# reallinshengxiang/Implementation-of-Rank-Algorithm-for-Mainstream-Recommender-Systems

Hardware: AMD Instinct MI355X
Metric: forward samples/sec at batch 4096 (DCN, DIN, BST) on 1/2/4/8 MI355X (higher is better)
Workload: dtype f32; 1 GPU; configs[2]: DIN forward, seq_len 50, emb_dim 32, batch 4096 per GPU; model=DIN, global_batch=4096, seq_len=50, emb_dim=32, tables=wechat_algo_data1 sizes (feedid 106445 rows), mode=eval, inputs resident in HBM, interaction_weights=frozen, parallelism=replicas x1, step=prepared single-kernel launch (rk_din_plan_launch)

## Files before the change

implementation-of-rank-algorithm-for-mainstream-recommender-systems_amd/csrc/din_fused.hip:

```cpp
#include <cstdlib>
#include <new>

#include "mlp_core.h"
#include "mlp_stream.h"

namespace rk {

typedef __attribute__((address_space(3))) void lds_void;
typedef __attribute__((address_space(1))) void glb_void;

#ifndef RK_DIN_HOIST
#define RK_DIN_HOIST 0
#endif

constexpr int kDinSegs = 32;
constexpr int kDinSegLdsOff = 528;
struct DinSegs {
  rk_segment s[kDinSegs];
};

struct DinArgs {
  DinSegs segs;
  uint8_t col_seg[256], col_off[256];
  const float* att_image;
  int nseg, width, q_col, att_col, l2_col0;
  const float* key_table;
  int64_t key_rows, ld_key;
  const int64_t* seq;
  int64_t ld_seq;
  int T;
  const int64_t* seq_len;
  int64_t batch;
  const float *w1, *b1, *w2, *b2, *w3, *b3;
  int use_softmax;
  int bal_nb;
  float* l2_part;
  unsigned* l2_count;
  float* l2_out;
  float l2_scale;
  uint32_t* flags;
  rk_mlp_layer L[RK_MLP_MAX_LAYERS];
  int nl;
  rk_epilogue head;
  int ld0, ld1;
  int epi_off;
  const float* epi_image;
};

template <int H>
struct DinLds {
  static constexpr int LDH = H + 4;
  static constexpr int WK = 0, WQK = WK + 64 * LDH, WQ = WQK + 64 * LDH, W2 = WQ + 64 * LDH;
  static constexpr int B1 = W2 + 32 * 68, B2 = B1 + 64, W3 = B2 + 32, U = W3 + 32, NORM = U + 16 * 64;
  static constexpr int BUF0 = NORM + 16;
};

#ifdef RK_DIN_PHASES
constexpr int kDinPhaseWG = 1024;
constexpr int kDinMarks = 9;
__device__ unsigned long long g_din_ts[kDinPhaseWG][kDinMarks];
__device__ unsigned long long g_din_wave[kDinPhaseWG][16];
__shared__ unsigned long long s_din_ts[kDinMarks];
__shared__ unsigned long long s_din_wave[16];
#define DIN_TS(i)                                \
  do {                                           \
    if (tid == 0) s_din_ts[i] = wall_clock64();  \
  } while (0)
#define DIN_TS_ENTRY()                                              \
  do {                                                              \
    if (tid < kDinMarks) s_din_ts[tid] = tid ? 0 : wall_clock64();  \
  } while (0)
__device__ __forceinline__ void din_marks_flush(int tid) {
  __syncthreads();
  if (blockIdx.x < kDinPhaseWG) {
    if (tid < kDinMarks) g_din_ts[blockIdx.x][tid] = s_din_ts[tid];
    if (tid < 16) g_din_wave[blockIdx.x][tid] = s_din_wave[tid];
  }
}
#else
#define DIN_TS(i) \
  do {            \
  } while (0)
#define DIN_TS_ENTRY() DIN_TS(0)
#endif

constexpr int kDinBalMax = 8;
constexpr int kDinBalClasses = 17;

__device__ __forceinline__ int wave_incl_scan(int v) {
  v += __builtin_amdgcn_update_dpp(0, v, 0x111, 0xf, 0xf, true);
  v += __builtin_amdgcn_update_dpp(0, v, 0x112, 0xf, 0xf, true);
  v += __builtin_amdgcn_update_dpp(0, v, 0x114, 0xf, 0xf, true);
  v += __builtin_amdgcn_update_dpp(0, v, 0x118, 0xf, 0xf, true);
  v += __builtin_amdgcn_update_dpp(0, v, 0x142, 0xa, 0xf, false);
  v += __builtin_amdgcn_update_dpp(0, v, 0x143, 0xc, 0xf, false);
  return v;
}

template <int H>
constexpr int din_pre_chunks() {
  return (16 + 34 + H) / 16 < 7 ? (16 + 34 + H) / 16 : 7;
}
static __shared__ unsigned s_din_rows_ready;
__device__ __forceinline__ void din_l2_handoff(float* l2_part, unsigned* l2_count, float* l2_out, float l2_scale,
                                               int64_t batch, const float* norms, int lane) {
  unsigned prev = 0;
  if (lane == 0) {
    float t = 0.f;
    for (int w = 0; w < kMlpRows; ++w) t += norms[w];
    const float old = __hip_atomic_exchange(l2_part + blockIdx.x, t, __ATOMIC_RELAXED, __HIP_MEMORY_SCOPE_AGENT);
    unsigned one = 1u;
    asm volatile("s_waitcnt vmcnt(0)" : "+v"(one) : "v"(old) : "memory");
    prev = __hip_atomic_fetch_add(l2_count, one, __ATOMIC_RELAXED, __HIP_MEMORY_SCOPE_AGENT);
  }
  prev = __builtin_amdgcn_readfirstlane(prev);
  if (prev == gridDim.x - 1) {
    float t = 0.f;
    for (int i = lane; i < (int)gridDim.x; i += 64)
      t += __hip_atomic_fetch_add(l2_part + i, 0.0f, __ATOMIC_RELAXED, __HIP_MEMORY_SCOPE_AGENT);
    t = wave_sum(t);
    if (lane == 0) {
      l2_out[0] = l2_scale * (t / (float)batch);
      __hip_atomic_store(l2_count, 0u, __ATOMIC_RELAXED, __HIP_MEMORY_SCOPE_AGENT);
    }
  }
#ifdef RK_DIN_PHASES
  if (lane == 0) s_din_ts[8] = wall_clock64();
#endif
}

struct DinL2Args {
  float* part;
  unsigned* count;
  float* out;
  float scale;
  int64_t batch;
};
static __shared__ DinL2Args s_din_l2;

template <class P, int H, bool WAIT, bool DMA>
struct DinRowsReady {
  static constexpr int kSideLayer = P::NL - 1;
  static_assert(P::NL >= 2 && P::nt(P::NL - 1) < kMlpWaves && P::tpw(P::NL - 1, kMlpWaves - 1) == 0,
                "the side layer leaves the last wave without a tile");
  __device__ void issue() const {}
  __device__ void operator()() const {
    if constexpr (DMA) asm volatile("s_waitcnt vmcnt(%0)" ::"n"(RK_STREAM_RING) : "memory");
    if constexpr (WAIT) {
      while (__builtin_amdgcn_readfirstlane(__hip_atomic_load(&s_din_rows_ready, __ATOMIC_RELAXED,
                                                              __HIP_MEMORY_SCOPE_WORKGROUP)) < (unsigned)kMlpWaves)
        __builtin_amdgcn_s_sleep(1);
      asm volatile("" ::: "memory");
    }
  }
  __device__ void side() const {
    if (__builtin_amdgcn_readfirstlane((int)threadIdx.x >> 6) != kMlpWaves - 1) return;
    const DinL2Args l2 = s_din_l2;
    if (!l2.part) return;
    extern __shared__ __attribute__((aligned(16))) float sm[];
    din_l2_handoff(l2.part, l2.count, l2.out, l2.scale, l2.batch, sm + DinLds<H>::NORM, (int)threadIdx.x & 63);
  }
};

template <int H, int NIT, class P, int KS = 0>
__global__ __launch_bounds__(kMlpThreads) void din_forward_kernel(DinArgs a) {
  using Ly = DinLds<H>;
  constexpr int NQ = H / 8;
  extern __shared__ __attribute__((aligned(16))) float sm[];
  float* const buf0 = sm + Ly::BUF0;
  float* const buf1 = buf0 + kMlpRows * a.ld0;
  uint8_t* const col_seg = reinterpret_cast<uint8_t*>(buf1 + kMlpRows * a.ld1);
  uint8_t* const col_off = col_seg + 256;
  rk_segment* const lsegs = reinterpret_cast<rk_segment*>(col_seg + kDinSegLdsOff);

  const int tid = threadIdx.x, lane = tid & 63, wave = tid >> 6;
  const int l32 = lane & 31, half = lane >> 5, hk = 4 * half;
  DIN_TS_ENTRY();

  static_assert(sizeof(rk_segment) % 4 == 0, "segment descriptor of whole words");
  const int seg_words = a.nseg * (int)(sizeof(rk_segment) / 4);
  uint8_t cs_v = 255, co_v = 0;
  int sw_v = 0;
  if (tid < 256) {
    cs_v = a.col_seg[tid];
    co_v = a.col_off[tid];
  }
  if (tid < seg_words) sw_v = reinterpret_cast<const int*>(&a.segs)[tid];

  const int64_t m0 = (int64_t)blockIdx.x * kMlpRows;
  const int ntiles_all = (a.T + 15) / 16;
  auto clamp_len = [&](int64_t len) { return len <= 0 ? 0 : (len >= a.T ? a.T : (int)len); };
  auto tiles_of = [&](int lc) { return lc ? (lc + 15) >> 4 : (a.use_softmax ? ntiles_all : 0); };
  int64_t* const kpre0 = reinterpret_cast<int64_t*>(col_seg + kDinSegLdsOff + sizeof(rk_segment) * kDinSegs);
  int64_t* const s_rows = kpre0 + 64 * kMlpRows;
  unsigned long long* const s_mask = reinterpret_cast<unsigned long long*>(s_rows + kMlpRows);
  int rows;
  int my_tiles = -1;
  int64_t my_len = 0;
  int64_t lv[NIT > 0 ? NIT : 1];
  int u0 = 0, UB = (int)a.batch, UG = (int)gridDim.x, ugl = (int)blockIdx.x;
  if constexpr (NIT == 1) {
    const int j = (int)blockIdx.x / (kMlpThreads / kMlpRows);
    u0 = j * kMlpThreads;
    UB = min(kMlpThreads, (int)(a.batch - u0));
    UG = (UB + kMlpRows - 1) / kMlpRows;
    ugl = (int)blockIdx.x - j * (kMlpThreads / kMlpRows);
  }
  if constexpr (NIT > 0) {
#pragma unroll
    for (int r = 0; r < NIT; ++r) {
      const int64_t i = u0 + tid + kMlpThreads * r;
      lv[r] = a.seq_len[i < a.batch ? i : a.batch - 1];
    }
  } else {
    rows = (int)min<int64_t>(kMlpRows, a.batch - m0);
    if (lane < rows) {
      my_len = a.seq_len[m0 + lane];
      my_tiles = tiles_of(clamp_len(my_len));
    }
  }

  static_assert(Ly::U % 4 == 0, "image of whole float4s");
  constexpr int kImg4 = Ly::U / 4, kPer = (kImg4 + kMlpThreads - 1) / kMlpThreads;
  f32x4_t v[kPer];
  if (a.att_image) {
#pragma unroll
    for (int r = 0; r < kPer; ++r) {
      const int i = tid + r * kMlpThreads;
      if (i < kImg4) v[r] = reinterpret_cast<const f32x4_t*>(a.att_image)[i];
    }
  }
  using Epi = std::conditional_t<std::is_void_v<P>, NoStage, StreamEpi<std::conditional_t<std::is_void_v<P>, StreamPlanK128, P>>>;
  Epi epi_img;
  const bool epi_dma = a.epi_image != nullptr;
#ifndef RK_DIN_EXP_NOEPI
  if constexpr (!std::is_void_v<P>)
    if (!epi_dma) epi_img.load(a.L, tid);
#endif
  auto image_to_lds = [&]() {
#ifndef RK_DIN_EXP_NOEPI
    if constexpr (!std::is_void_v<P>)
      if (!epi_dma) epi_img.store(sm + a.epi_off, tid);
#endif
    if (a.att_image) {
#pragma unroll
      for (int r = 0; r < kPer; ++r) {
        const int i = tid + r * kMlpThreads;
        if (i < kImg4) reinterpret_cast<f32x4_t*>(sm)[i] = v[r];
      }
    } else {
      for (int i = tid; i < 64 * H; i += kMlpThreads) {
        const int j = i / H, h = i % H;
        const float* r = a.w1 + (int64_t)j * 4 * H;
        sm[Ly::WQ + j * Ly::LDH + h] = r[h] + r[2 * H + h];
        sm[Ly::WK + j * Ly::LDH + h] = r[H + h] - r[2 * H + h];
        sm[Ly::WQK + j * Ly::LDH + h] = r[3 * H + h];
      }
      for (int i = tid; i < 32 * 64; i += kMlpThreads) sm[Ly::W2 + (i / 64) * 68 + (i % 64)] = a.w2[i];
      if (tid < 64) sm[Ly::B1 + tid] = a.b1[tid];
      if (tid < 32) {
        sm[Ly::B2 + tid] = a.b2[tid];
        sm[Ly::W3 + tid] = a.w3[tid];
      }
    }
  };
  if (tid < 256) {
    col_seg[tid] = cs_v;
    col_off[tid] = co_v;
  }
  if (tid < seg_words) reinterpret_cast<int*>(lsegs)[tid] = sw_v;
  uint32_t* flags = a.flags;

  const int wp = pad64(a.width);
  constexpr int kColIt = 4;
  int64_t kidx = 0;
  float cval[kColIt];
  auto gather_issue = [&](int64_t bs, bool lv_, int nt_) {
    if (lv_ && lane < 16 * nt_ && lane < a.T) kidx = a.seq[bs * a.ld_seq + lane];
    int64_t cidx[kColIt];
    int cseg[kColIt];
#pragma unroll
    for (int i = 0; i < kColIt; ++i) {
      const int c = lane + 64 * i;
      cseg[i] = (lv_ && c < a.width) ? col_seg[c] : 255;
      cidx[i] = bs;
      if (cseg[i] != 255 && lsegs[cseg[i]].idx) cidx[i] = lsegs[cseg[i]].idx[bs * lsegs[cseg[i]].idx_stride];
    }
#pragma unroll
    for (int i = 0; i < kColIt; ++i) {
      const int c = lane + 64 * i;
      cval[i] = 0.f;
      if (cseg[i] != 255) {
        const rk_segment& g = lsegs[cseg[i]];
        if (g.idx && (cidx[i] < 0 || cidx[i] >= g.rows))
          flag_oob(flags);
        else
          cval[i] = g.src[cidx[i] * g.src_ld + col_off[c]];
      }
    }
  };
  auto gather_store = [&](float* rowp, int64_t* kslot) {
    kslot[lane] = kidx;
#pragma unroll
    for (int i = 0; i < kColIt; ++i) {
      const int c = lane + 64 * i;
      if (c < wp) rowp[c] = cval[i];
    }
  };

  if constexpr (NIT == 0) {
    asm volatile("s_waitcnt lgkmcnt(0)\n\ts_barrier" ::: "memory");
    const int tiles_w = __builtin_amdgcn_readlane(my_tiles, wave);
    gather_issue(m0 + wave, wave < rows, tiles_w);
    image_to_lds();
// ... 633 lines not shown
```

implementation-of-rank-algorithm-for-mainstream-recommender-systems_amd/csrc/mlp_core.h:

```cpp
#pragma once

#include <type_traits>

#include "common.h"

namespace rk {

#ifndef RK_MLP_EPI_PRIO
#define RK_MLP_EPI_PRIO 1
#endif
#ifndef RK_MLP_SYNC
#define RK_MLP_SYNC 1
#endif
#ifndef RK_MLP_EARLY_RING
#define RK_MLP_EARLY_RING 0
#endif
#ifndef RK_MLP_EP_LANES16
#define RK_MLP_EP_LANES16 0
#endif
#ifndef RK_MLP_UNIFORM_PREP
#define RK_MLP_UNIFORM_PREP 0
#endif

constexpr int kMlpRows = 16;
// ... 191 lines not shown
        const int cA = min(c + 1, kchunks - 1);
#pragma unroll
        for (int t = 0; t < RT; ++t)
          ab[(s + 1) & 1][t] = *reinterpret_cast<const f32x4_t*>(arow + 16 * t * ldin + 16 * cA);
        __builtin_amdgcn_sched_barrier(0);
#pragma unroll
        for (int e = 0; e < 4; ++e)
#pragma unroll
          for (int j = 0; j < TPW; ++j)
#pragma unroll
            for (int t = 0; t < RT; ++t) acc[j][t] = mfma16(ab[s & 1][t][e], P.ring[s * TPW + j][e], acc[j][t]);
        if constexpr (decltype(refill)::value) {
          const int cn = min(c + PD, kchunks - 1);
#pragma unroll
          for (int j = 0; j < TPW; ++j)
            P.ring[s * TPW + j] = *reinterpret_cast<const f32x4_t*>(P.wrow[j] + kFragStep * cn);
        }
      }
      __builtin_amdgcn_sched_barrier(0);
    }
  };
  int c0 = 0;
  for (; c0 + PD < kchunks; c0 += PD) {
    cycle(c0, PD, std::true_type{});
#if RK_MLP_SYNC
    if ((c0 + PD) % kMlpSyncChunks == 0) mlp_sync_barrier();
#endif
  }
  if (kchunks - c0 == PD) {
    cycle(c0, PD, std::false_type{});
  } else {
    cycle(c0, kchunks - c0, std::false_type{});
    __builtin_amdgcn_s_waitcnt(0x0F70);
  }
  next();

#ifdef RK_MLP_PHASES
  if (wave == 0 && lane == 0) s_mlp_marks[dbg_mark] = clock64() - dbg_t0;
  if (lane == 0 && dbg_mark / 4 < 4) s_mlp_wave_marks[dbg_mark / 4][wave][0] = (unsigned)(clock64() - dbg_t0);
#endif
#if RK_MLP_EPI_PRIO
  __builtin_amdgcn_s_setprio(2);
#endif
  float* const store = STORE ? L.store : nullptr;
  const int64_t ld_store = L.ld_store;
  auto epilogue = [&](auto DICE, auto RES) {
#pragma unroll
    for (int j = 0; j < TPW; ++j) {
      const int n = 16 * (wave + kMlpWaves * j) + li;
      const bool real = n < L.n;
      const ColEpi ep = ep_bcast(P.ep[j], lane);
      float res[RT][4];
#pragma unroll
      for (int t = 0; t < RT; ++t)
#pragma unroll
        for (int r = 0; r < 4; ++r) res[t][r] = RES ? out[(16 * t + (lane >> 4) * 4 + r) * ldout + n] : 0.f;
#pragma unroll
      for (int t = 0; t < RT; ++t)
#pragma unroll
        for (int r = 0; r < 4; ++r) {
          const int row = 16 * t + (lane >> 4) * 4 + r;
          const float v = col_apply(L, ep, DICE, acc[j][t][r], RES, res[t][r]);
          const float z = real ? v : 0.f;
          out[row * ldout + n] = z;
          if constexpr (STORE)
            if (store && real && row < rows) store[(m0 + row) * ld_store + n] = z;
        }
    }
  };
  const bool dice = L.act == RK_ACT_DICE;
  if (L.residual != 0) {
    if (dice)
      epilogue(std::true_type{}, std::true_type{});
    else
      epilogue(std::false_type{}, std::true_type{});
  } else {
    if (dice)
      epilogue(std::true_type{}, std::false_type{});
    else
      epilogue(std::false_type{}, std::false_type{});
  }
#ifdef RK_MLP_PHASES
  if (lane == 0 && dbg_mark / 4 < 4) s_mlp_wave_marks[dbg_mark / 4][wave][1] = (unsigned)(clock64() - dbg_t0);
#endif
}

__device__ __forceinline__ void mlp_lds_barrier() { asm volatile("s_waitcnt lgkmcnt(0)\n\ts_barrier" ::: "memory"); }

struct NoStage {
  __device__ void issue() const {}
  __device__ void operator()() const {}
  __device__ void side() const {}
};
template <class I, class F>
struct TwoPhaseStage {
  I i;
  F f;
  __device__ void issue() { i(); }
  __device__ void operator()() { f(); }
  __device__ void side() {}
};
template <class E, class I, class F, class S>
struct StagedStage {
  static constexpr bool kEarly = true;
  E e;
  I i;
  F f;
  S s;
  __device__ void early() { e(); }
  __device__ void issue() { i(); }
  __device__ void operator()() { f(); }
  __device__ void side() { s(); }
};
template <class E, class I, class F, class S>
__device__ __forceinline__ StagedStage<E, I, F, S> staged(E e, I i, F f, S s) {
  return StagedStage<E, I, F, S>{e, i, f, s};
}
template <class T, class = void>
struct stage_has_early : std::false_type {};
template <class T>
struct stage_has_early<T, std::void_t<decltype(T::kEarly)>> : std::true_type {};
template <class T, class = void>
struct stage_side_layer {
  static constexpr int value = -1;
};
template <class T>
struct stage_side_layer<T, std::void_t<decltype(T::kSideLayer)>> {
  static constexpr int value = T::kSideLayer;
};
template <class T, class = void>
struct stage_pre_chunks {
  static constexpr int value = 0;
};
template <class T>
struct stage_pre_chunks<T, std::void_t<decltype(T::kPreChunks)>> {
  static constexpr int value = T::kPreChunks;
};
template <int KS, class S>
struct PreChunks : S {
  static constexpr int kPreChunks = KS;
};
template <class T, class = void>
struct stage_ring_early {
  static constexpr int value = -1;
};
template <class T>
struct stage_ring_early<T, std::void_t<decltype(T::kRingEarly)>> {
  static constexpr int value = T::kRingEarly;
};
template <int N, class S>
struct RingEarly : S {
  static constexpr int kRingEarly = N;
};
template <int N, class S>
__device__ __forceinline__ RingEarly<N, S> ring_early(S s) {
  return RingEarly<N, S>{s};
}
template <int L, class S>
struct SideAt : S {
  static constexpr int kSideLayer = L;
};
template <int L, class S>
__device__ __forceinline__ SideAt<L, S> side_at(S s) {
  return SideAt<L, S>{s};
}
template <class I, class F>
__device__ __forceinline__ TwoPhaseStage<I, F> two_phase(I i, F f) {
  return TwoPhaseStage<I, F>{i, f};
}
template <class F>
__device__ __forceinline__ auto finish_only(F f) {
  return two_phase([] {}, f);
}

template <int RT = 1, bool STORE = false, class Stage = NoStage>
__device__ __forceinline__ void mlp_rows(const rk_mlp_layer* __restrict__ layers, int nl, int K0, float* buf0,
                                         int ld0, float* buf1, int ld1, int64_t m0, int rows,
                                         const rk_epilogue& h, float* y, int64_t ldy, int tid,
                                         Stage stage = Stage(), const float* lds_partial = nullptr,
                                         const int64_t* row_ids = nullptr) {
  const int lane = tid & 63, wave = __builtin_amdgcn_readfirstlane(tid >> 6);
  LayerPipe pipe;
  auto prepare = [&](int l) {
    const int nt = pad64(layers[l].n) / 16;
    const int kch = pad64(l ? layers[l - 1].n : K0) / 16;
#if RK_MLP_UNIFORM_PREP
    if (wave < nt) pipe.prepare_any(layers[l], kch, wave + kMlpWaves < nt, wave, lane);
#else
    if (wave + kMlpWaves < nt)
      pipe.prepare<2, 4>(layers[l], kch, wave, lane);
    else if (wave < nt)
      pipe.prepare<1, 8>(layers[l], kch, wave, lane);
#endif
  };
#if RK_MLP_EARLY_RING
  auto prepare_ring = [&](int l) {
    const int nt = pad64(layers[l].n) / 16;
    const int kch = pad64(layers[l - 1].n) / 16;
    if (wave + kMlpWaves < nt)
      pipe.prepare_ring<2, 4>(layers[l], kch, wave, lane);
    else if (wave < nt)
      pipe.prepare_ring<1, 8>(layers[l], kch, wave, lane);
  };
  auto prepare_ep = [&](int l) {
    const int nt = pad64(layers[l].n) / 16;
    if (wave + kMlpWaves < nt)
      pipe.prepare_ep<2>(layers[l], wave, lane);
    else if (wave < nt)
      pipe.prepare_ep<1>(layers[l], wave, lane);
  };
#endif
  const int Kh = nl ? layers[nl - 1].n : K0;
  const bool hpre = h.head_w != nullptr && Kh <= 128;
  float hw[2] = {0.f, 0.f};
  float hp = 0.f;
  auto head_prefetch = [&]() {
    if (!hpre) return;
#pragma unroll
    for (int c = 0; c < 2; ++c)
      if (lane + 64 * c < Kh) hw[c] = h.head_w[lane + 64 * c];
    if (wave < rows && h.head_partial && !lds_partial) hp = h.head_partial[row_ids ? row_ids[wave] : m0 + wave];
  };
#ifdef RK_MLP_PHASES
  const unsigned long long t_start = clock64();
#endif
  stage.issue();
  __builtin_amdgcn_sched_barrier(0);
  if (nl > 0) prepare(0);
  if (nl <= 1) head_prefetch();
  MLP_MARK(4 * RK_MLP_MAX_LAYERS - 4, t_start);
  stage();
  mlp_lds_barrier();
  MLP_MARK(4 * RK_MLP_MAX_LAYERS, t_start);
  int Kp = pad64(K0);
  for (int l = 0; l < nl; ++l) {
    const unsigned long long t0 =
#ifdef RK_MLP_PHASES
        clock64();
#else
        0;
#endif
    const rk_mlp_layer& L = layers[l];
    const int ntiles = pad64(L.n) / 16;
    const float* in = (l & 1) ? buf1 : buf0;
    float* out = (l & 1) ? buf0 : buf1;
    const int ldin = (l & 1) ? ld1 : ld0, ldout = (l & 1) ? ld0 : ld1;
#if RK_MLP_EARLY_RING
    auto next = [&] {
      if (l + 1 < nl) prepare_ring(l + 1);
    };
#else
    auto next = [] {};
#endif
    if (wave + kMlpWaves < ntiles) {
      mlp_layer<2, RT, 4, STORE>(pipe, L, in, ldin, out, ldout, Kp, wave, lane, m0, rows, next, 4 * l, t0);
    } else if (wave < ntiles) {
      mlp_layer<1, RT, 8, STORE>(pipe, L, in, ldin, out, ldout, Kp, wave, lane, m0, rows, next, 4 * l, t0);
    } else {
#if RK_MLP_SYNC
      for (int i = 0; i < (Kp / 16 - 1) / kMlpSyncChunks; ++i) mlp_sync_barrier();
#endif
      next();
    }
    MLP_MARK(4 * l + 1, t0);
#if RK_MLP_EARLY_RING
    if (l + 1 < nl) prepare_ep(l + 1);
#else
    if (l + 1 < nl) prepare(l + 1);
#endif
    if (l + 2 == nl) head_prefetch();
    MLP_MARK(4 * l + 2, t0);
    mlp_lds_barrier();
#if RK_MLP_EPI_PRIO
    __builtin_amdgcn_s_setprio(0);
#endif
    MLP_MARK(4 * l + 3, t0);
    Kp = pad64(L.n);
  }
  const float* fin = (nl & 1) ? buf1 : buf0;
  const int ldf = (nl & 1) ? ld1 : ld0;
  const int K = nl ? layers[nl - 1].n : K0;
  if (h.head_w) {
    for (int r = wave; r < rows; r += kMlpWaves) {
      const bool pre = hpre && r == wave;
      float p = 0.f;
      if (pre) {
#pragma unroll
        for (int c = 0; c < 2; ++c)
          if (lane + 64 * c < K) p = fmaf(fin[r * ldf + lane + 64 * c], hw[c], p);
      } else {
        for (int n = lane; n < K; n += 64) p = fmaf(fin[r * ldf + n], h.head_w[n], p);
      }
      p = wave_sum(p);
      if (lane == 0) {
        const int64_t m = row_ids ? row_ids[r] : m0 + r;
        float logit = p + h.head_b[0];
        if (lds_partial)
          logit = lds_partial[r] + logit;
        else if (h.head_partial)
          logit = (pre ? hp : h.head_partial[m]) + logit;
        if (h.fm1) {
          if (h.head_aux) h.head_aux[m] = logit;
          logit = h.fm1[m] * h.final_w[0] + h.fm2[m] * h.final_w[1] + logit * h.final_w[2] + h.final_b[0];
        }
        if (h.head_logit) h.head_logit[m] = logit;
        if (h.head_prob) h.head_prob[m] = 1.0f / (1.0f + expf(-logit));
// ... 15 lines not shown
```

implementation-of-rank-algorithm-for-mainstream-recommender-systems_amd/csrc/mlp_stream.h:

```cpp
#pragma once

#include <type_traits>
#include <utility>

#include "mlp_core.h"

namespace rk {

#ifndef RK_STREAM_RING
#define RK_STREAM_RING 8
#endif
#ifndef RK_STREAM_EPI
#define RK_STREAM_EPI 2
#endif
#ifndef RK_STREAM_SPLITACC
#define RK_STREAM_SPLITACC 0
#endif
#ifndef RK_STREAM_FLAGS
#define RK_STREAM_FLAGS 0
#endif
#ifndef RK_STREAM_NT
#define RK_STREAM_NT 0
#endif
#ifndef RK_STREAM_REFILL_GROUP
#define RK_STREAM_REFILL_GROUP 4
#endif
#ifndef RK_STREAM_RING_EARLY
#define RK_STREAM_RING_EARLY 2
#endif
constexpr int kStreamStaticLds = 64;
#if RK_STREAM_FLAGS
static __shared__ unsigned rk_stream_ready[RK_MLP_MAX_LAYERS];
#endif

template <int B, int E, class F>
__device__ __forceinline__ void static_for(F&& f) {
  if constexpr (B < E) {
    f(std::integral_constant<int, B>{});
    static_for<B + 1, E>(f);
  }
}

template <int KC0_, int... NT_>
struct StreamPlan {
  static constexpr int NL = sizeof...(NT_);
  static constexpr int KC0 = KC0_;
  static constexpr int nt(int l) {
    constexpr int v[] = {NT_...};
    return v[l];
  }
  static constexpr int kc(int l) { return l == 0 ? KC0 : nt(l - 1); }
  static constexpr int tpw(int l, int w) { return w < nt(l) ? (nt(l) - 1 - w) / 16 + 1 : 0; }
  static constexpr int base(int l, int w) {
    int b = 0;
    for (int i = 0; i < l; ++i) b += tpw(i, w) * kc(i);
    return b;
  }
  static constexpr int layer_of(int g, int w) {
    int l = 0;
    while (l + 1 < NL && base(l + 1, w) <= g) ++l;
    return l;
  }
  static constexpr bool same_class(int a, int b) {
    for (int l = 0; l < NL; ++l)
      if (tpw(l, a) != tpw(l, b)) return false;
    return true;
  }
  static constexpr int rep(int w) {
    int r = 0;
    while (!same_class(r, w)) ++r;
    return r;
  }
  static constexpr int epi_off(int l) {
    int o = 0;
    for (int i = 0; i < l; ++i) o += 16 * nt(i) * 8;
    return o;
  }
  static constexpr int epi_floats() { return epi_off(NL); }
  static constexpr int epi_cols() { return epi_off(NL) / 8; }
  static_assert(NL >= 1 && NL <= RK_MLP_MAX_LAYERS, "layer count");
  static_assert(epi_off(NL) / 8 <= 2 * kMlpThreads, "epilogue image: two columns per thread at most");
};

__device__ __forceinline__ ColEpi resolve_epi(const rk_mlp_layer& L, ColEpi r) {
  r.bias = L.bias ? r.bias : 0.f;
  r.pre_s = L.pre_scale ? r.pre_s : 1.f;
  r.pre_b = L.pre_scale ? r.pre_b : 0.f;
  r.post_s = L.post_scale ? r.post_s : 1.f;
  r.post_b = L.post_scale ? r.post_b : 0.f;
  if (L.act != RK_ACT_DICE)
    r.alpha = L.act == RK_ACT_RELU ? 0.f : L.act == RK_ACT_LEAKY ? L.slope : L.act == RK_ACT_PRELU ? r.alpha : 1.f;
  return r;
}

template <bool DICE>
__device__ __forceinline__ float apply_epi(const ColEpi& e, float z) {
  z = z + e.bias;
  z = z * e.pre_s + e.pre_b;
  if constexpr (DICE)
    z = dice_apply(z, e.act_s, e.act_b, e.alpha);
  else
    z = z > 0.f ? z : z * e.alpha;
  return z * e.post_s + e.post_b;
}

enum StreamEpiMode {
  kEpiLdsHere = 0,
  kEpiLdsCaller = 1,
  kEpiRegs = 2,
};

template <class P>
struct StreamEpi {
  ColEpi e[2];
  static constexpr int kCols = (P::epi_cols() + kMlpThreads - 1) / kMlpThreads;
  __device__ __forceinline__ void load(const rk_mlp_layer* __restrict__ layers, int tid) {
#pragma unroll
    for (int k = 0; k < kCols; ++k) {
      const int i = tid + kMlpThreads * k;
      int l = 0;
#pragma unroll
      for (int q = 1; q < P::NL; ++q) l = i >= P::epi_off(q) / 8 ? q : l;
      rk_mlp_layer L = layers[0];
#pragma unroll
      for (int q = 1; q < P::NL; ++q)
        if (l == q) L = layers[q];
      const int n = i - P::epi_off(l) / 8;
      e[k] = resolve_epi(L, col_epi(L, n < L.n ? n : 0));
    }
  }
  __device__ __forceinline__ void store(float* __restrict__ img, int tid) const {
#pragma unroll
    for (int k = 0; k < kCols; ++k) {
      const int i = tid + kMlpThreads * k;
      if (i < P::epi_cols()) {
        f32x4_t* d = reinterpret_cast<f32x4_t*>(img + 8 * i);
        d[0] = (f32x4_t){e[k].bias, e[k].pre_s, e[k].pre_b, e[k].act_s};
        d[1] = (f32x4_t){e[k].act_b, e[k].alpha, e[k].post_s, e[k].post_b};
      }
    }
  }
};

constexpr int side_chunk(int KC, int k) {
  const int step = KC / 4 > 0 ? KC / 4 : 1;
  const int c = (KC > 2 ? 2 : KC - 1) + step * k;
  return c < KC - 1 ? c : KC - 1;
}
constexpr int side_first_pos(int KC, int c) {
  for (int k = 0; k < 4; ++k)
    if (side_chunk(KC, k) == c) return k;
  return 4;
}
constexpr int side_last_pos(int KC, int c) {
  for (int k = 3; k >= 0; --k)
    if (side_chunk(KC, k) == c) return k;
  return -1;
}

template <class P, int W, int EPI, int RT, bool IP0, class Stage>
__device__ __forceinline__ void mlp_stream_class(const rk_mlp_layer* __restrict__ layers, float* buf0, int ld0,
                                                 float* buf1, int ld1, float* epi, int64_t m0, int rows,
                                                 const rk_epilogue& h, int tid, int wave, Stage& stage,
                                                 const float* lds_partial, const int64_t* row_ids,
                                                 const float* lds_fm) {
  constexpr int R = RK_STREAM_RING;
  constexpr int NL = P::NL;
  constexpr int TOT = P::base(NL, W);
  const int lane = tid & 63, li = lane & 15, kq = 4 * (lane >> 4);
  f32x4_t ring[R];

  auto issue = [&](auto G) {
    constexpr int g = G;
    if constexpr (g < TOT) {
      constexpr int l = P::layer_of(g, W);
      constexpr int T = P::tpw(l, W);
      constexpr int i = g - P::base(l, W), c = i / T, j = i % T;
      const rk_mlp_layer& L = layers[l];
      const float* p = L.w + ((int64_t)(wave + kMlpWaves * j) * (L.ldw / 16) + c) * kFragStep;
#if RK_STREAM_NT
      ring[g % R] = __builtin_nontemporal_load(reinterpret_cast<const f32x4_t*>(p + 4 * lane));
#else
      ring[g % R] = *reinterpret_cast<const f32x4_t*>(p + 4 * lane);
#endif
    }
  };

  const int Kh = layers[NL - 1].n;
  const bool hpre = h.head_w != nullptr && Kh <= 128;
  float hw[2] = {0.f, 0.f};
  float hp = 0.f;
  auto head_prefetch = [&]() {
    if (!hpre) return;
#pragma unroll
    for (int c = 0; c < 2; ++c)
      if (lane + 64 * c < Kh) hw[c] = h.head_w[lane + 64 * c];
    if (wave < rows && h.head_partial && !lds_partial) hp = h.head_partial[row_ids ? row_ids[wave] : m0 + wave];
  };

#ifdef RK_MLP_PHASES
  const unsigned long long t_start = clock64();
#endif
  StreamEpi<P> ep_stage;
  constexpr bool kEarly = stage_has_early<Stage>::value;
  constexpr int kSideL = stage_side_layer<Stage>::value >= 0 ? stage_side_layer<Stage>::value : (NL > 1 ? 1 : 0);
  ColEpi epr[2];
  auto load_epr = [&](auto LI) {
    constexpr int l = LI;
    if constexpr (l < NL) {
      const rk_mlp_layer& L = layers[l];
#pragma unroll
      for (int j = 0; j < P::tpw(l, W); ++j) {
        const int n = 16 * (wave + kMlpWaves * j) + li;
        epr[j] = col_epi(L, n < L.n ? n : 0);
      }
    }
  };
  if constexpr (kEarly) {
    stage.early();
    __builtin_amdgcn_sched_barrier(0);
  } else {
    stage.issue();
    if constexpr (EPI == kEpiLdsHere) ep_stage.load(layers, tid);
    __builtin_amdgcn_sched_barrier(0);
  }
  constexpr int kRE = stage_ring_early<Stage>::value >= 0 ? stage_ring_early<Stage>::value : RK_STREAM_RING_EARLY;
  constexpr int R0 = kEarly ? (kRE < R ? kRE : R) : R;
  static_for<0, R0>([&](auto G) {
    issue(G);
    __builtin_amdgcn_sched_barrier(0);
  });
  if constexpr (kEarly) {
    stage.issue();
    if constexpr (EPI == kEpiLdsHere) ep_stage.load(layers, tid);
    __builtin_amdgcn_sched_barrier(0);
    static_for<R0, R>([&](auto G) {
      issue(G);
      __builtin_amdgcn_sched_barrier(0);
    });
  }
  if constexpr (EPI == kEpiRegs) load_epr(std::integral_constant<int, 0>{});
  if constexpr (NL == 1) head_prefetch();
  MLP_MARK(4 * RK_MLP_MAX_LAYERS - 4, t_start);
  stage();
  constexpr int KS = stage_pre_chunks<Stage>::value;
  constexpr int T0 = P::tpw(0, W);
  static_assert(KS == 0 || (KS < kMlpSyncChunks && KS < P::kc(0) && kSideL != 0 && !(RK_STREAM_SPLITACC && T0 == 1) &&
                            RT == 1 && !IP0),
                "pre-barrier chunks: no lockstep barrier or side work among them");
  static_assert(RT == 1 || RT == 2, "one or two 16-row tiles");
  f32x4_t acc0[T0 > 0 ? T0 : 1];
  if constexpr (KS > 0 && T0 > 0) {
#pragma unroll
    for (int j = 0; j < T0; ++j) acc0[j] = (f32x4_t){0.f, 0.f, 0.f, 0.f};
    const float* arow = buf0 + li * ld0 + kq;
    f32x4_t ab[2];
    ab[0] = *reinterpret_cast<const f32x4_t*>(arow);
    static_for<0, KS>([&](auto CI) {
      constexpr int c = CI;
      if constexpr (c + 1 < KS) ab[(c + 1) & 1] = *reinterpret_cast<const f32x4_t*>(arow + 16 * (c + 1));
      __builtin_amdgcn_sched_barrier(0);
      static_for<0, 4>([&](auto EI) {
        constexpr int e = EI;
        static_for<0, T0>([&](auto JI) {
          constexpr int j = JI;
          acc0[j] = mfma16(ab[c & 1][e], ring[(c * T0 + j) % R][e], acc0[j]);
        });
      });
      static_for<0, T0>([&](auto JI) {
        constexpr int j = JI;
        issue(std::integral_constant<int, c * T0 + j + R>{});
      });
      __builtin_amdgcn_sched_barrier(0);
    });
  }
  if constexpr (EPI == kEpiLdsHere) ep_stage.store(epi, tid);
#if RK_STREAM_FLAGS
  if (tid < NL) rk_stream_ready[tid] = 0u;
#endif
  mlp_lds_barrier();
  MLP_MARK(4 * RK_MLP_MAX_LAYERS, t_start);

  static_for<0, NL>([&](auto LI) {
    constexpr int l = LI;
    constexpr int T = P::tpw(l, W), KC = P::kc(l), B0 = P::base(l, W);
#ifdef RK_MLP_PHASES
    const unsigned long long t0 = clock64();
#endif
    const rk_mlp_layer& L = layers[l];
    constexpr bool kSync = !(stage_side_layer<Stage>::value == l && P::nt(l) < kMlpWaves);
    constexpr bool kIn1 = IP0 ? (l > 0 && !(l & 1)) : (l & 1);
    constexpr bool kOut1 = IP0 ? (l & 1) : !(l & 1);
    const float* in = kIn1 ? buf1 : buf0;
    float* out = kOut1 ? buf1 : buf0;
    const int ldin = kIn1 ? ld1 : ld0, ldout = kOut1 ? ld1 : ld0;
    if constexpr (T == 0) {
      if constexpr (l == kSideL) stage.side();
#if RK_MLP_SYNC
      if constexpr (kSync)
        static_for<0, (KC - 1) / kMlpSyncChunks>([&](auto) { mlp_sync_barrier(); });
#endif
      if constexpr (IP0 && l == 0) mlp_lds_barrier();
    } else {
      constexpr int CB = l == 0 ? KS : 0;
      f32x4_t acc[T][RT];
#pragma unroll
      for (int j = 0; j < T; ++j) {
#pragma unroll
        for (int t = 0; t < RT; ++t) {
          if constexpr (CB > 0)
            acc[j][t] = acc0[j];
          else
            acc[j][t] = (f32x4_t){0.f, 0.f, 0.f, 0.f};
        }
      }
      constexpr bool kSplit = RK_STREAM_SPLITACC && T == 1 && RT == 1;
      f32x4_t acc_odd = {0.f, 0.f, 0.f, 0.f};
      const float* arow = in + li * ldin + kq;
      unsigned ready = 0u;
      auto wait_chunk = [&](int c) {
#if RK_STREAM_FLAGS
        if constexpr (l > 0) {
          if (!((ready >> c) & 1u)) {
            do {
              ready = __builtin_amdgcn_readfirstlane(
                  __hip_atomic_load(&rk_stream_ready[l - 1], __ATOMIC_RELAXED, __HIP_MEMORY_SCOPE_WORKGROUP));
            } while (!((ready >> c) & 1u));
            asm volatile("" ::: "memory");
          }
        }
#endif
      };
      f32x4_t ab[2][RT];
      wait_chunk(CB);
#pragma unroll
      for (int t = 0; t < RT; ++t) ab[CB & 1][t] = *reinterpret_cast<const f32x4_t*>(arow + 16 * t * ldin + 16 * CB);
      static_for<CB, KC>([&](auto CI) {
        constexpr int c = CI;
        if constexpr (c + 1 < KC) {
          wait_chunk(c + 1);
#pragma unroll
          for (int t = 0; t < RT; ++t)
            ab[(c + 1) & 1][t] = *reinterpret_cast<const f32x4_t*>(arow + 16 * t * ldin + 16 * (c + 1));
        }
        __builtin_amdgcn_sched_barrier(0);
        static_for<0, 4>([&](auto EI) {
          constexpr int e = EI;
          static_for<0, T>([&](auto JI) {
            constexpr int j = JI;
            static_for<0, RT>([&](auto TI) {
              constexpr int t = TI;
              if constexpr (kSplit && (e & 1))
                acc_odd = mfma16(ab[c & 1][t][e], ring[(B0 + c * T + j) % R][e], acc_odd);
              else
                acc[j][t] = mfma16(ab[c & 1][t][e], ring[(B0 + c * T + j) % R][e], acc[j][t]);
            });
          });
        });
        {
          constexpr int CG = RK_STREAM_REFILL_GROUP / T > 1 ? RK_STREAM_REFILL_GROUP / T : 1;
          if constexpr ((c - CB + 1) % CG == 0 || c + 1 == KC) {
            constexpr int c0 = c - (c - CB) % CG;
            static_for<c0 * T, (c + 1) * T>([&](auto GI) {
              constexpr int g = GI;
              issue(std::integral_constant<int, B0 + g + R>{});
            });
          }
        }
        __builtin_amdgcn_sched_barrier(0);
        if constexpr (l == kSideL) {
          constexpr int kFirst = side_first_pos(KC, c), kLast = side_last_pos(KC, c);
          if constexpr (kFirst <= kLast) {
            const int pos = wave >> 2;
            if (pos >= kFirst && pos <= kLast) stage.side();
            __builtin_amdgcn_sched_barrier(0);
          }
        }
#if RK_MLP_SYNC
        if constexpr (kSync && (c + 1) % kMlpSyncChunks == 0 && c + 1 < KC) mlp_sync_barrier();
#endif
      });
      if constexpr (kSplit) acc[0][0] += acc_odd;
      if constexpr (IP0 && l == 0) mlp_lds_barrier();
      MLP_MARK(4 * l, t0);
#ifdef RK_MLP_PHASES
      if (lane == 0 && l < 4) s_mlp_wave_marks[l][wave][0] = (unsigned)(clock64() - t0);
#endif
#if RK_MLP_EPI_PRIO
      __builtin_amdgcn_s_setprio(2);
#endif
      const float* img = epi + P::epi_off(l);
      auto epilogue = [&](auto DICE) {
#pragma unroll
        for (int j = 0; j < T; ++j) {
          const int n = 16 * (wave + kMlpWaves * j) + li;
          const bool real = n < L.n;
          ColEpi e;
          if constexpr (EPI == kEpiRegs) {
            e = resolve_epi(L, epr[j]);
          } else {
            const f32x4_t p0 = *reinterpret_cast<const f32x4_t*>(img + 8 * n);
            const f32x4_t p1 = *reinterpret_cast<const f32x4_t*>(img + 8 * n + 4);
            e.bias = p0[0];
            e.pre_s = p0[1];
            e.pre_b = p0[2];
            e.act_s = p0[3];
            e.act_b = p1[0];
            e.alpha = p1[1];
            e.post_s = p1[2];
            e.post_b = p1[3];
          }
#pragma unroll
          for (int t = 0; t < RT; ++t) {
#pragma unroll
            for (int r = 0; r < 4; ++r) {
              const int row = 16 * t + (lane >> 4) * 4 + r;
              const float z = apply_epi<decltype(DICE)::value>(e, acc[j][t][r]);
              out[row * ldout + n] = real ? z : 0.f;
            }
          }
        }
      };
      if (L.act == RK_ACT_DICE)
        epilogue(std::true_type{});
      else
        epilogue(std::false_type{});
#if RK_STREAM_FLAGS
      if constexpr (l + 1 < NL) {
        asm volatile("s_waitcnt lgkmcnt(0)" ::: "memory");
        unsigned bits = 0u;
#pragma unroll
        for (int j = 0; j < T; ++j) bits |= 1u << (wave + kMlpWaves * j);
        if (lane == 0) __hip_atomic_fetch_or(&rk_stream_ready[l], bits, __ATOMIC_RELAXED, __HIP_MEMORY_SCOPE_WORKGROUP);
      }
#endif
#ifdef RK_MLP_PHASES
      if (lane == 0 && l < 4) s_mlp_wave_marks[l][wave][1] = (unsigned)(clock64() - t0);
#endif
    }
    MLP_MARK(4 * l + 1, t0);
    if constexpr (EPI == kEpiRegs) load_epr(std::integral_constant<int, l + 1>{});
    if constexpr (l + 2 == NL) head_prefetch();
    MLP_MARK(4 * l + 2, t0);
    if constexpr (!RK_STREAM_FLAGS || l + 1 == NL) mlp_lds_barrier();
    MLP_MARK(4 * l + 3, t0);
#if RK_MLP_EPI_PRIO
    if constexpr (T > 0) __builtin_amdgcn_s_setprio(0);
#endif
  });

  constexpr bool kFin1 = IP0 ? ((NL - 1) & 1) : (NL & 1);
  const float* fin = kFin1 ? buf1 : buf0;
  const int ldf = kFin1 ? ld1 : ld0;
  const int K = Kh;
  if (h.head_w) {
    for (int r = wave; r < rows; r += kMlpWaves) {
      const bool pre = hpre && r == wave;
      float p = 0.f;
      if (pre) {
#pragma unroll
        for (int c = 0; c < 2; ++c)
          if (lane + 64 * c < K) p = fmaf(fin[r * ldf + lane + 64 * c], hw[c], p);
      } else {
        for (int n = lane; n < K; n += 64) p = fmaf(fin[r * ldf + n], h.head_w[n], p);
      }
      p = wave_sum(p);
      if (lane == 0) {
        const int64_t m = row_ids ? row_ids[r] : m0 + r;
        float logit = p + h.head_b[0];
        if (lds_partial)
          logit = lds_partial[r] + logit;
        else if (h.head_partial)
          logit = (pre ? hp : h.head_partial[m]) + logit;
        if (h.fm1) {
          if (h.head_aux) h.head_aux[m] = logit;
          const float f1 = lds_fm ? lds_fm[r] : h.fm1[m], f2 = lds_fm ? lds_fm[kMlpRows * RT + r] : h.fm2[m];
          logit = f1 * h.final_w[0] + f2 * h.final_w[1] + logit * h.final_w[2] + h.final_b[0];
        }
        if (h.head_logit) h.head_logit[m] = logit;
        if (h.head_prob) h.head_prob[m] = 1.0f / (1.0f + expf(-logit));
      }
    }
  }
}

template <class P, int EPI = kEpiRegs, int RT = 1, bool IP0 = false, class Stage = NoStage>
__device__ __forceinline__ void mlp_stream_rows(const rk_mlp_layer* __restrict__ layers, float* buf0, int ld0,
                                                float* buf1, int ld1, float* epi, int64_t m0, int rows,
                                                const rk_epilogue& h, int tid, Stage stage = Stage(),
                                                const float* lds_partial = nullptr,
                                                const int64_t* row_ids = nullptr, const float* lds_fm = nullptr) {
  const int wave = __builtin_amdgcn_readfirstlane(tid >> 6);
  static_for<0, kMlpWaves>([&](auto WI) {
    constexpr int w = WI;
    if constexpr (P::rep(w) == w) {
      bool mine = true;
#pragma unroll
      for (int l = 0; l < P::NL; ++l) mine = mine && P::tpw(l, wave) == P::tpw(l, w);
      if (mine)
        mlp_stream_class<P, w, EPI, RT, IP0>(layers, buf0, ld0, buf1, ld1, epi, m0, rows, h, tid, wave, stage,
                                         lds_partial, row_ids, lds_fm);
    }
  });
}

using StreamPlanK64 = StreamPlan<4, 32, 16, 8>;
using StreamPlanK80 = StreamPlan<5, 32, 16, 8>;
using StreamPlanK128 = StreamPlan<8, 32, 16, 8>;
using StreamPlanK192 = StreamPlan<12, 32, 16, 8>;
using StreamPlanK256 = StreamPlan<16, 32, 16, 8>;
using StreamPlanTail512 = StreamPlan<32, 16, 8>;
using StreamPlanK960 = StreamPlan<60, 32, 16, 8>;

enum StreamPlanId { kStreamNone = 0, kStreamK64, kStreamK128, kStreamK192, kStreamK256, kStreamTail512 };
int stream_plan_for(const rk_mlp_layer* layers, int nlayers, int K0);
int stream_plan_epi_floats(int id);

}
```

Before: 109.5 million samples/s.

## Split L2 grid handoff into staged side steps interleaved with layer-1 chunks

Replaces the single-shot L2 regularizer handoff, previously run by the last wave at the last MLP layer, with four staged steps. They are placed at chunk boundaries of layers 0 and 1, just after ring refills, so the atomic exchange, counter increment and final reduction loads overlap with MFMA work. Each global atomic's latency is hidden behind compute instead of stalling at the tail. The change also drops the per-chunk sync barriers in the last layer (free layer) and adds phase timestamps for profiling. The risks are extra register pressure from the held state, and correctness if the barrier removal breaks ordering.

```diff
diff --git a/implementation-of-rank-algorithm-for-mainstream-recommender-systems_amd/csrc/din_fused.hip b/implementation-of-rank-algorithm-for-mainstream-recommender-systems_amd/csrc/din_fused.hip
--- a/implementation-of-rank-algorithm-for-mainstream-recommender-systems_amd/csrc/din_fused.hip
+++ b/implementation-of-rank-algorithm-for-mainstream-recommender-systems_amd/csrc/din_fused.hip
@@ -8,6 +8,8 @@
 
 typedef __attribute__((address_space(3))) void lds_void;
 typedef __attribute__((address_space(1))) void glb_void;
+typedef __attribute__((address_space(1))) float glb_float;
+typedef __attribute__((address_space(1))) unsigned glb_uint;
 
 #ifndef RK_DIN_HOIST
 #define RK_DIN_HOIST 0
@@ -57,7 +59,7 @@
 
 #ifdef RK_DIN_PHASES
 constexpr int kDinPhaseWG = 1024;
-constexpr int kDinMarks = 9;
+constexpr int kDinMarks = 13;
 __device__ unsigned long long g_din_ts[kDinPhaseWG][kDinMarks];
 __device__ unsigned long long g_din_wave[kDinPhaseWG][16];
 __shared__ unsigned long long s_din_ts[kDinMarks];
@@ -73,7 +75,8 @@
 __device__ __forceinline__ void din_marks_flush(int tid) {
   __syncthreads();
   if (blockIdx.x < kDinPhaseWG) {
-    if (tid < kDinMarks) g_din_ts[blockIdx.x][tid] = s_din_ts[tid];
+    if (tid < 10) g_din_ts[blockIdx.x][tid] = s_din_ts[tid];
+    if (tid >= 10 && tid < kDinMarks) g_din_ts[blockIdx.x][tid] = s_stream_last_ts[tid - 10];
     if (tid < 16) g_din_wave[blockIdx.x][tid] = s_din_wave[tid];
   }
 }
@@ -101,6 +104,9 @@
 constexpr int din_pre_chunks() {
   return (16 + 34 + H) / 16 < 7 ? (16 + 34 + H) / 16 : 7;
 }
+#ifndef RK_DIN_FREE_LAST
+#define RK_DIN_FREE_LAST 1
+#endif
 static __shared__ unsigned s_din_rows_ready;
 __device__ __forceinline__ void din_l2_handoff(float* l2_part, unsigned* l2_count, float* l2_out, float l2_scale,
                                                int64_t batch, const float* norms, int lane) {
@@ -125,7 +131,10 @@
     }
   }
 #ifdef RK_DIN_PHASES
-  if (lane == 0) s_din_ts[8] = wall_clock64();
+  if (lane == 0) {
+    s_din_ts[8] = wall_clock64();
+    s_din_ts[9] = prev == gridDim.x - 1;
+  }
 #endif
 }
 
@@ -140,9 +149,84 @@
 
 template <class P, int H, bool WAIT, bool DMA>
 struct DinRowsReady {
-  static constexpr int kSideLayer = P::NL - 1;
-  static_assert(P::NL >= 2 && P::nt(P::NL - 1) < kMlpWaves && P::tpw(P::NL - 1, kMlpWaves - 1) == 0,
-                "the side layer leaves the last wave without a tile");
+#if RK_DIN_FREE_LAST
+  static constexpr int kFreeLayer = P::NL - 1;
+#endif
+  static constexpr int kSideSteps = 4, kSideWave = kMlpWaves - 1;
+  static constexpr int kHeld = 4;
+  static constexpr int side_step_layer(int s) { return s == 0 ? 0 : 1; }
+  static constexpr int side_step_chunk(int s) { return s == 0 ? -1 : 8 * s - 5; }
+  static_assert(P::NL >= 2 && P::kc(1) >= 24 && RK_STREAM_RING == 8 && (RK_STREAM_REFILL_GROUP == 4 || RK_STREAM_REFILL_GROUP == 1),
+                "the steps sit behind refills of layer 1, a ring apart");
+  struct SideState {
+    glb_float* l2_part;
+    glb_uint* l2_count;
+    float old;
+    unsigned prev;
+    float part[kHeld];
+  };
+  template <class T>
+  static __device__ __forceinline__ T uniform_global(const void* p) {
+    const uint64_t v = reinterpret_cast<uint64_t>(p);
+    const uint32_t lo = __builtin_amdgcn_readfirstlane((uint32_t)v), hi = __builtin_amdgcn_readfirstlane((uint32_t)(v >> 32));
+    return (T)(((uint64_t)hi << 32) | lo);
+  }
+  template <int S>
+  __device__ __forceinline__ void side_step(SideState& st) const {
+    extern __shared__ __attribute__((aligned(16))) float sm[];
+    const int lane = (int)threadIdx.x & 63;
+    if constexpr (S == 0) {
+      st.l2_part = uniform_global<glb_float*>(s_din_l2.part);
+      st.l2_count = uniform_global<glb_uint*>(s_din_l2.count);
+    }
+    glb_float* const l2_part = st.l2_part;
+    if (!l2_part) return;
+    const int grid = (int)gridDim.x;
+    if constexpr (S == 0) {
+      if (lane == 0) {
+        const float* norms = sm + DinLds<H>::NORM;
+        float t = 0.f;
+        for (int w = 0; w < kMlpRows; ++w) t += norms[w];
+        st.old = __hip_atomic_exchange(l2_part + blockIdx.x, t, __ATOMIC_RELAXED, __HIP_MEMORY_SCOPE_AGENT);
+      }
+    } else if constexpr (S == 1) {
+      if (lane == 0) {
+        glb_uint* count = st.l2_count;
+        asm volatile("" : "+v"(count) : "v"(st.old) : "memory");
+        st.prev = __hip_atomic_fetch_add(count, 1u, __ATOMIC_RELAXED, __HIP_MEMORY_SCOPE_AGENT);
+      }
+    } else if constexpr (S == 2) {
+      st.prev = __builtin_amdgcn_readfirstlane(st.prev);
+      if (st.prev == (unsigned)grid - 1u) {
+#pragma unroll
+        for (int k = 0; k < kHeld; ++k) {
+          const int i = lane + 64 * k;
+          st.part[k] = 0.f;
+          if (i < grid) st.part[k] = __hip_atomic_fetch_add(l2_part + i, 0.0f, __ATOMIC_RELAXED, __HIP_MEMORY_SCOPE_AGENT);
+        }
+      }
+    } else {
+      if (st.prev == (unsigned)grid - 1u) {
+        float t = 0.f;
+#pragma unroll
+        for (int k = 0; k < kHeld; ++k) t += st.part[k];
+        for (int i = lane + 64 * kHeld; i < grid; i += 64)
+          t += __hip_atomic_fetch_add(l2_part + i, 0.0f, __ATOMIC_RELAXED, __HIP_MEMORY_SCOPE_AGENT);
+        t = wave_sum(t);
+        if (lane == 0) {
+          const DinL2Args l2 = s_din_l2;
+          ((glb_float*)l2.out)[0] = l2.scale * (t / (float)l2.batch);
+          __hip_atomic_store(st.l2_count, 0u, __ATOMIC_RELAXED, __HIP_MEMORY_SCOPE_AGENT);
+        }
+      }
+#ifdef RK_DIN_PHASES
+      if (lane == 0) {
+        s_din_ts[8] = wall_clock64();
+        s_din_ts[9] = st.prev == (unsigned)grid - 1u;
+      }
+#endif
+    }
+  }
   __device__ void issue() const {}
   __device__ void operator()() const {
     if constexpr (DMA) asm volatile("s_waitcnt vmcnt(%0)" ::"n"(RK_STREAM_RING) : "memory");
@@ -153,13 +237,7 @@
       asm volatile("" ::: "memory");
     }
   }
-  __device__ void side() const {
-    if (__builtin_amdgcn_readfirstlane((int)threadIdx.x >> 6) != kMlpWaves - 1) return;
-    const DinL2Args l2 = s_din_l2;
-    if (!l2.part) return;
-    extern __shared__ __attribute__((aligned(16))) float sm[];
-    din_l2_handoff(l2.part, l2.count, l2.out, l2.scale, l2.batch, sm + DinLds<H>::NORM, (int)threadIdx.x & 63);
-  }
+  __device__ void side() const {}
 };
 
 template <int H, int NIT, class P, int KS = 0>
diff --git a/implementation-of-rank-algorithm-for-mainstream-recommender-systems_amd/csrc/mlp_core.h b/implementation-of-rank-algorithm-for-mainstream-recommender-systems_amd/csrc/mlp_core.h
--- a/implementation-of-rank-algorithm-for-mainstream-recommender-systems_amd/csrc/mlp_core.h
+++ b/implementation-of-rank-algorithm-for-mainstream-recommender-systems_amd/csrc/mlp_core.h
@@ -367,6 +367,25 @@
 struct RingEarly : S {
   static constexpr int kRingEarly = N;
 };
+template <class T, class = void>
+struct stage_free_layer {
+  static constexpr int value = -1;
+};
+template <class T>
+struct stage_free_layer<T, std::void_t<decltype(T::kFreeLayer)>> {
+  static constexpr int value = T::kFreeLayer;
+};
+struct NoSideState {};
+template <class T, class = void>
+struct stage_side_steps {
+  static constexpr int value = 0;
+  using State = NoSideState;
+};
+template <class T>
+struct stage_side_steps<T, std::void_t<decltype(T::kSideSteps)>> {
+  static constexpr int value = T::kSideSteps;
+  using State = typename T::SideState;
+};
 template <int N, class S>
 __device__ __forceinline__ RingEarly<N, S> ring_early(S s) {
   return RingEarly<N, S>{s};
diff --git a/implementation-of-rank-algorithm-for-mainstream-recommender-systems_amd/csrc/mlp_stream.h b/implementation-of-rank-algorithm-for-mainstream-recommender-systems_amd/csrc/mlp_stream.h
--- a/implementation-of-rank-algorithm-for-mainstream-recommender-systems_amd/csrc/mlp_stream.h
+++ b/implementation-of-rank-algorithm-for-mainstream-recommender-systems_amd/csrc/mlp_stream.h
@@ -31,6 +31,18 @@
 constexpr int kStreamStaticLds = 64;
 #if RK_STREAM_FLAGS
 static __shared__ unsigned rk_stream_ready[RK_MLP_MAX_LAYERS];
+#endif
+
+#ifdef RK_DIN_PHASES
+__shared__ unsigned long long s_stream_last_ts[3];
+#define STREAM_LAST_TS(i)                                                    \
+  do {                                                                       \
+    if (tid == kMlpThreads - 64) s_stream_last_ts[i] = wall_clock64();       \
+  } while (0)
+#else
+#define STREAM_LAST_TS(i) \
+  do {                    \
+  } while (0)
 #endif
 
 template <int B, int E, class F>
@@ -156,6 +168,20 @@
   for (int k = 3; k >= 0; --k)
     if (side_chunk(KC, k) == c) return k;
   return -1;
+}
+
+template <class P, class Stage, int W, int KS>
+constexpr bool side_steps_placed() {
+  int pl = -1, pc = -2;
+  for (int s = 0; s < stage_side_steps<Stage>::value; ++s) {
+    const int l = Stage::side_step_layer(s), c = Stage::side_step_chunk(s);
+    if (l < 0 || l >= P::NL || P::tpw(l, W) == 0) return false;
+    if (c != -1 && (c < (l == 0 ? KS : 0) || c >= P::kc(l))) return false;
+    if (l < pl || (l == pl && c <= pc)) return false;
+    pl = l;
+    pc = c;
+  }
+  return true;
 }
 
 template <class P, int W, int EPI, int RT, bool IP0, class Stage>
@@ -203,7 +229,8 @@
 #endif
   StreamEpi<P> ep_stage;
   constexpr bool kEarly = stage_has_early<Stage>::value;
-  constexpr int kSideL = stage_side_layer<Stage>::value >= 0 ? stage_side_layer<Stage>::value : (NL > 1 ? 1 : 0);
+  constexpr int kSideL = stage_side_steps<Stage>::value > 0 ? -1
+                         : stage_side_layer<Stage>::value >= 0 ? stage_side_layer<Stage>::value : (NL > 1 ? 1 : 0);
   ColEpi epr[2];
   auto load_epr = [&](auto LI) {
     constexpr int l = LI;
@@ -280,6 +307,25 @@
 #endif
   mlp_lds_barrier();
   MLP_MARK(4 * RK_MLP_MAX_LAYERS, t_start);
+  STREAM_LAST_TS(0);
+
+  constexpr int kSteps = stage_side_steps<Stage>::value;
+  [[maybe_unused]] typename stage_side_steps<Stage>::State side_state{};
+  auto side_steps_at = [&](auto LI, auto CI) {
+    if constexpr (kSteps > 0) {
+      if constexpr (P::rep(Stage::kSideWave) == W) {
+        static_assert(side_steps_placed<P, Stage, W, KS>(), "side steps: ascending, at chunks of tiled layers");
+        static_for<0, kSteps>([&](auto SI) {
+          constexpr int s = SI;
+          if constexpr (Stage::side_step_layer(s) == decltype(LI)::value &&
+                        Stage::side_step_chunk(s) == decltype(CI)::value) {
+            if (wave == Stage::kSideWave) stage.template side_step<s>(side_state);
+            __builtin_amdgcn_sched_barrier(0);
+          }
+        });
+      }
+    }
+  };
 
   static_for<0, NL>([&](auto LI) {
     constexpr int l = LI;
@@ -287,8 +333,11 @@
 #ifdef RK_MLP_PHASES
     const unsigned long long t0 = clock64();
 #endif
+    if constexpr (l == NL - 1) STREAM_LAST_TS(1);
+    side_steps_at(LI, std::integral_constant<int, -1>{});
     const rk_mlp_layer& L = layers[l];
-    constexpr bool kSync = !(stage_side_layer<Stage>::value == l && P::nt(l) < kMlpWaves);
+    constexpr bool kSync = !(stage_side_layer<Stage>::value == l && P::nt(l) < kMlpWaves) &&
+                           stage_free_layer<Stage>::value != l;
     constexpr bool kIn1 = IP0 ? (l > 0 && !(l & 1)) : (l & 1);
     constexpr bool kOut1 = IP0 ? (l & 1) : !(l & 1);
     const float* in = kIn1 ? buf1 : buf0;
@@ -368,6 +417,7 @@
           }
         }
         __builtin_amdgcn_sched_barrier(0);
+        side_steps_at(LI, CI);
         if constexpr (l == kSideL) {
           constexpr int kFirst = side_first_pos(KC, c), kLast = side_last_pos(KC, c);
           if constexpr (kFirst <= kLast) {
@@ -442,6 +492,7 @@
     if constexpr (EPI == kEpiRegs) load_epr(std::integral_constant<int, l + 1>{});
     if constexpr (l + 2 == NL) head_prefetch();
     MLP_MARK(4 * l + 2, t0);
+    if constexpr (l == NL - 1) STREAM_LAST_TS(2);
     if constexpr (!RK_STREAM_FLAGS || l + 1 == NL) mlp_lds_barrier();
     MLP_MARK(4 * l + 3, t0);
 #if RK_MLP_EPI_PRIO
```

Measured after the change: 113.0 million samples/s (median of 6 runs). 1.03x the previous value.
